# optuna/optuna

Measured on AMD Instinct MI355X. Metric: sampler suggest()/sec at 10k-trial history, 20-dim space, higher is better.
Workload: dtype fp64; 1 GPU; model=TPESampler multivariate Parzen-KDE + EI, history_trials=10000, dims=20, n_ei_candidates=24, parallelism=single, hip_kernels=True

## Files before the change

### optuna_amd/_hip/csrc/hipcore.hip

```cpp
#include "hip_common.h"

#include "gp_logei.h"
#include "mo_host.h"
#include "mo_rank.h"
#include "tpe_host.h"
#include "truncnorm_ops.h"

PYBIND11_MODULE(_hipcore, m) {
    m.doc() = "optuna_amd MI355X (gfx950) HIP kernels: TPE parzen fit + mixture "
              "log-pdf, truncnorm device library";
    m.def("available", &available);
    m.def("device_count", &device_count);
    m.def("log_gauss_mass", &log_gauss_mass);
    m.def("truncnorm_ppf", &truncnorm_ppf);
    m.def("truncnorm_logpdf", &truncnorm_logpdf);
    m.def("nondomination_rank", &nondomination_rank, py::arg("vals"),
          py::arg("n_below"));
    m.def("hv3d", &hv3d, py::arg("pts"), py::arg("ref_x"), py::arg("ref_y"),
          py::arg("ref_z"));
    py::class_<GpLogEiSession>(m, "GpLogEiSession")
        .def(py::init<int64_t, int64_t, int64_t, int64_t, int64_t, int64_t,
                      double, double, double>(),
             py::arg("X_ptr"), py::arg("alpha_ptr"), py::arg("cinv_ptr"),
             py::arg("eta_ptr"), py::arg("N"), py::arg("D"), py::arg("scale"),
             py::arg("stab_noise"), py::arg("threshold"))
        .def("eval", &GpLogEiSession::eval, py::arg("x"), py::arg("with_grad"));
    py::class_<Hssp3dSession>(m, "Hssp3dSession")
        .def(py::init<const arr_f64&, double, double, double>(), py::arg("cand"),
             py::arg("ref_x"), py::arg("ref_y"), py::arg("ref_z"))
        .def("round", &Hssp3dSession::round, py::arg("sx"), py::arg("sxz"),
             py::arg("sy"), py::arg("syz"), py::arg("syr"))
        .def("run", &Hssp3dSession::run, py::arg("subset_size"));
    m.def("hssp3d_contrib", &hssp3d_contrib, py::arg("cand"), py::arg("sx"),
          py::arg("sxz"), py::arg("sy"), py::arg("syz"), py::arg("syr"),
          py::arg("ref_x"), py::arg("ref_y"), py::arg("ref_z"));
    m.def("hv4d", &hv4d, py::arg("pts"), py::arg("ref_w"), py::arg("ref_x"),
          py::arg("ref_y"), py::arg("ref_z"));
    m.def("hssp4d_contrib", &hssp4d_contrib, py::arg("cand"), py::arg("sw"),
          py::arg("sx"), py::arg("sy"), py::arg("syz"), py::arg("syrw"),
          py::arg("syrx"), py::arg("ref_w"), py::arg("ref_x"), py::arg("ref_y"),
          py::arg("ref_z"));
    py::class_<Hssp4dSession>(m, "Hssp4dSession")
        .def(py::init<const arr_f64&, double, double, double, double>(),
             py::arg("cand"), py::arg("ref_w"), py::arg("ref_x"),
             py::arg("ref_y"), py::arg("ref_z"))
        .def("run", &Hssp4dSession::run, py::arg("subset_size"));
    m.attr("HSSP4D_MAX_SUBSET") = py::int_(HSSP4_MAX_K);
    m.def("kde_logpdf", &kde_logpdf, py::arg("obs"), py::arg("sorted_pos"),
          py::arg("logw"), py::arg("alow"), py::arg("ahigh"), py::arg("steps"),
          py::arg("n_choices"), py::arg("prior_weight"),
          py::arg("x"), py::arg("xedges"),
          py::arg("consider_endpoints") = false, py::arg("magic_clip") = true);
    m.def("tpe_below_kernels", &tpe_below_kernels, py::arg("obs"),
          py::arg("alow"), py::arg("ahigh"), py::arg("consider_endpoints"),
          py::arg("consider_magic_clip"), py::arg("active"));
    py::class_<TpeDeviceHistory>(m, "TpeDeviceHistory")
        .def(py::init<int64_t>(), py::arg("dims"))
        .def_property_readonly("n_rows", &TpeDeviceHistory::n_rows)
        .def("append", &TpeDeviceHistory::append, py::arg("block"))
        .def("upload_sorted", &TpeDeviceHistory::upload_sorted, py::arg("cols"))
        .def("insert_sorted", &TpeDeviceHistory::insert_sorted, py::arg("pos"),
             py::arg("rows"))
        .def_property_readonly("n_sorted", &TpeDeviceHistory::n_sorted)
        .def("insert_sorted_by_value", &TpeDeviceHistory::insert_sorted_by_value,
             py::arg("first_row"), py::arg("n_new"))
        .def("sorted_index", &TpeDeviceHistory::sorted_index)
        .def("set_domain", &TpeDeviceHistory::set_domain, py::arg("alow"),
             py::arg("ahigh"), py::arg("steps"), py::arg("n_choices"))
        .def("fused_prepare", &TpeDeviceHistory::fused_prepare, py::arg("excl"),
             py::arg("n_above"), py::arg("logw") = arr_f64(),
             py::arg("w_num") = 0, py::arg("w_start") = 1.0,
             py::arg("w_step") = 0.0, py::arg("log_total") = 0.0,
             py::arg("prior_weight") = 1.0,
             py::arg("consider_endpoints") = false,
             py::arg("magic_clip") = true)
        .def("fused_score", &TpeDeviceHistory::fused_score, py::arg("excl"),
             py::arg("n_above"), py::arg("x"), py::arg("xedges"),
             py::arg("bmu"), py::arg("bsig"), py::arg("bw"),
             py::arg("logw") = arr_f64(), py::arg("w_num") = 0,
             py::arg("w_start") = 1.0, py::arg("w_step") = 0.0,
             py::arg("log_total") = 0.0, py::arg("prior_weight") = 1.0,
             py::arg("consider_endpoints") = false,
             py::arg("magic_clip") = true, py::arg("return_parts") = false)
        .def("score", &TpeDeviceHistory::score, py::arg("sorted_rows"),
             py::arg("pos"), py::arg("n_above"), py::arg("logw"), py::arg("alow"),
             py::arg("ahigh"), py::arg("steps"), py::arg("n_choices"),
             py::arg("prior_weight"), py::arg("x"), py::arg("xedges"),
             py::arg("consider_endpoints") = false,
             py::arg("magic_clip") = true,
             py::arg("extras_raw") = arr_f64(),
             py::arg("extras_sorted") = arr_f64(),
             py::arg("extras_sorted_idx") = arr_i32(),
             py::arg("per_dim") = false);
}
```

### optuna_amd/_hip/csrc/tpe_host.h

```cpp
#pragma once

#include "hip_common.h"
#include "tpe_below_host.h"
#include "tpe_fused_kernels.h"
#include "tpe_kernels.h"

static void launch_mix_logpdf(hipStream_t st, const double* d_x,
                              const double* d_xedges, const double* d_c1,
                              const double* d_c2, const double* d_c3,
                              const double* d_logw, const double* d_steps,
                              const double* d_nchoices, double cat_base,
                              int64_t K, int64_t D, int64_t S, double* d_out,
                              double* d_scratch) {
    const int block = 256;
    const size_t shmem = (4 * (size_t)D + 2 * block) * sizeof(double);
    const int64_t n_chunks = mix_n_chunks(K);
    if (n_chunks <= 1) {
        hipLaunchKernelGGL(k_mix_logpdf, dim3((unsigned)S), dim3(block), shmem, st,
                           d_x, d_xedges, d_c1, d_c2, d_c3, d_logw, d_steps,
                           d_nchoices, cat_base, K, D, d_out);
        return;
    }
    double* d_part_m = d_scratch;
    double* d_part_s = d_scratch + (size_t)n_chunks * S;
    hipLaunchKernelGGL(k_mix_logpdf_partial, dim3((unsigned)S, (unsigned)n_chunks),
                       dim3(block), shmem, st, d_x, d_xedges, d_c1, d_c2, d_c3,
                       d_logw, d_steps, d_nchoices, cat_base, K, D, MIX_CHUNK,
                       d_part_m, d_part_s);
    hipLaunchKernelGGL(k_mix_logpdf_merge, dim3((unsigned)S), dim3(64), 0, st,
                       d_part_m, d_part_s, n_chunks, S, d_out);
}

py::array_t<double> kde_logpdf(const arr_f64& obs, const arr_i64& sorted_pos,
                               const arr_f64& logw, const arr_f64& alow,
                               const arr_f64& ahigh, const arr_f64& steps,
                               const arr_f64& n_choices, double prior_weight,
// ... 387 lines not shown

    void fused_prepare(const arr_i32& excl, int64_t n_above, const arr_f64& logw,
                       int64_t w_num, double w_start, double w_step,
                       double log_total, double prior_weight,
                       bool consider_endpoints, bool magic_clip) {
        check_fit_args("fused_prepare", excl, n_above, logw);
        g_ws.begin_uploads();
        launch_fit(excl, n_above, logw, w_num, w_start, w_step, log_total,
                   prior_weight, consider_endpoints, magic_clip,
                   true);
    }

    py::object fused_score(const arr_i32& excl, int64_t n_above,
                                    const arr_f64& x, const arr_f64& xedges,
                                    const arr_f64& bmu, const arr_f64& bsig,
                                    const arr_f64& bw, const arr_f64& logw,
                                    int64_t w_num, double w_start,
                                    double w_step, double log_total,
                                    double prior_weight,
                                    bool consider_endpoints, bool magic_clip,
                                    bool return_parts) {
        check_fit_args("fused_score", excl, n_above, logw);
        if (x.ndim() != 2 || x.shape(1) != D_ || bmu.ndim() != 2 ||
            bmu.shape(1) != D_ || bsig.ndim() != 2 || bsig.shape(1) != D_)
            throw std::runtime_error("fused_score: shape mismatch");
        const int64_t S = x.shape(0);
        const int64_t Kb = bmu.shape(0);
        const int64_t K = n_above + 1;
        if (S < 1 || Kb < 1 || Kb > FUSED_MAX_BELOW || bsig.shape(0) != Kb ||
            (int64_t)bw.size() != Kb ||
            (has_steps_ && (int64_t)xedges.size() != 2 * S * D_))
            throw std::runtime_error("fused_score: shape mismatch");

        hipStream_t st = g_ws.get_stream();
        g_ws.begin_uploads();
        if (!prepared_matches(excl, n_above, logw, w_num, w_start, w_step,
                              log_total, prior_weight, consider_endpoints,
                              magic_clip))
            launch_fit(excl, n_above, logw, w_num, w_start, w_step, log_total,
                       prior_weight, consider_endpoints, magic_clip,
                       false);

        const size_t n_x = (size_t)S * D_;
        const size_t n_b = (size_t)Kb * D_;
        const int64_t n_as = (K + SCORE_SLICE - 1) / SCORE_SLICE;
        const int64_t pass_dims = std::min<int64_t>(D_, SCORE_DC);
        const int below_slice = (int)std::max<int64_t>(
            1, std::min<int64_t>(SCORE_SLICE, SCORE_SLICE * SCORE_WAVES / pass_dims));
        const int64_t n_bs = (Kb + below_slice - 1) / below_slice;
        const size_t n_part = (size_t)(n_as + n_bs) * S;
        WsLayout L;
        const auto s_x = L.add<double>(n_x);
        const auto s_bmu = L.add<double>(n_b), s_bsig = L.add<double>(n_b);
        const auto s_bw = L.add<double>(Kb);
        const auto s_xedges = L.add<double>(has_steps_ ? 2 * n_x : 0);
        const size_t up_bytes = L.bytes();
        const auto s_part_m = L.add<double>(n_part), s_part_s = L.add<double>(n_part);
        char* base = g_ws.ensure_bytes(L.bytes());
        double *d_x = s_x.in(base), *d_bmu = s_bmu.in(base),
               *d_bsig = s_bsig.in(base), *d_bw = s_bw.in(base),
               *d_xedges = s_xedges.in(base), *d_part_m = s_part_m.in(base),
               *d_part_s = s_part_s.in(base);
        {
            char* h = g_ws.stage(up_bytes, st);
            memcpy(s_x.in(h), x.data(), n_x * 8);
            memcpy(s_bmu.in(h), bmu.data(), n_b * 8);
            memcpy(s_bsig.in(h), bsig.data(), n_b * 8);
            memcpy(s_bw.in(h), bw.data(), (size_t)Kb * 8);
            if (has_steps_) memcpy(s_xedges.in(h), xedges.data(), 2 * n_x * 8);
            HIP_CHECK(hipMemcpyAsync(base, h, up_bytes, hipMemcpyHostToDevice, st));
        }

        const CoefLayout C(K, D_, excl.size());
        const double* d_logw = C.logw.in(coef_.ptr);
        const int64_t n_groups = (S + SCORE_CAND - 1) / SCORE_CAND;
        hipLaunchKernelGGL(k_fused_score,
                           dim3((unsigned)(n_as + n_bs), (unsigned)n_groups),
                           dim3(SCORE_SLICE * SCORE_WAVES), 0, st, d_x, d_xedges,
                           C.c1.in(coef_.ptr), C.c2.in(coef_.ptr),
                           C.c3.in(coef_.ptr), d_logw, K, n_as,
                           d_bmu, d_bsig, d_bw, Kb, below_slice, domain_.ptr,
                           has_steps_ ? 1 : 0,
                           D_, S, d_part_m, d_part_s);
        const double* h_out =
            reinterpret_cast<const double*>(g_ws.stage(3 * (size_t)S * 8, st));
        hipLaunchKernelGGL(k_fused_merge, dim3((unsigned)S), dim3(64), 0, st,
                           d_part_m, d_part_s, n_as, n_bs, S,
                           const_cast<double*>(h_out));
        if (return_parts) {
            py::array_t<double> parts({(int64_t)3, S});
            py::array_t<double> lw(K);
            HIP_CHECK(hipMemcpyAsync(lw.mutable_data(), d_logw, (size_t)K * 8,
                                     hipMemcpyDeviceToHost, st));
            HIP_CHECK(hipStreamSynchronize(st));
            HIP_CHECK(hipGetLastError());
            memcpy(parts.mutable_data(), h_out, 3 * (size_t)S * 8);
            return py::make_tuple(parts, lw);
        }
        py::array_t<double> out(S);
        HIP_CHECK(hipStreamSynchronize(st));
        HIP_CHECK(hipGetLastError());
        memcpy(out.mutable_data(), h_out, (size_t)S * 8);
        return out;
    }

  private:
    struct PreparedFit {
        bool valid = false;
        int64_t n = 0, n_sorted = 0, Na = 0, w_num = 0;
        double w_start = 0.0, w_step = 0.0, log_total = 0.0, prior_weight = 0.0;
        bool consider_endpoints = false, magic_clip = false;
        std::vector<int32_t> excl;
        std::vector<double> logw;
    };

    void check_fit_args(const char* who, const arr_i32& excl, int64_t Na,
                        const arr_f64& logw) const {
        const std::string w(who);
        if (!sorted_valid_) throw std::runtime_error(w + " before upload_sorted");
        if (!domain_.ptr) throw std::runtime_error(w + " before set_domain");
        if (has_categorical_)
            throw std::runtime_error(w + ": categorical dims unsupported");
        const int64_t E = excl.size();
        const int64_t Nv = n_sorted_;
        if (E > FUSED_MAX_EXCL || Na < 0 || Na > Nv || Na + E < Nv ||
            (logw.size() > 0 && (int64_t)logw.size() != Na + 1))
            throw std::runtime_error(w + ": shape mismatch");
        const int32_t* ex = excl.data();
        for (int64_t e = 0; e < E; ++e)
            if (ex[e] < 0 || ex[e] >= n_ || (e > 0 && ex[e] <= ex[e - 1]))
                throw std::runtime_error(w + ": excl must be sorted table rows");
    }

    bool prepared_matches(const arr_i32& excl, int64_t Na, const arr_f64& logw,
                          int64_t w_num, double w_start, double w_step,
                          double log_total, double prior_weight,
                          bool consider_endpoints, bool magic_clip) const {
        const PreparedFit& p = prep_;
        const double a[4] = {w_start, w_step, log_total, prior_weight};
        const double b[4] = {p.w_start, p.w_step, p.log_total, p.prior_weight};
        return p.valid && p.n == n_ && p.n_sorted == n_sorted_ && p.Na == Na &&
               p.w_num == w_num && memcmp(a, b, sizeof(a)) == 0 &&
               p.consider_endpoints == consider_endpoints &&
               p.magic_clip == magic_clip &&
               p.excl.size() == (size_t)excl.size() &&
               (p.excl.empty() ||
                memcmp(p.excl.data(), excl.data(), p.excl.size() * 4) == 0) &&
               p.logw.size() == (size_t)logw.size() &&
               (p.logw.empty() ||
                memcmp(p.logw.data(), logw.data(), p.logw.size() * 8) == 0);
    }

    struct CoefLayout {
        WsLayout L;
        WsSlot<double> c1, c2, c3, logw;
        WsSlot<int32_t> excl;
        CoefLayout(int64_t K, int64_t D, int64_t E)
            : c1(L.add<double>((size_t)K * D)), c2(L.add<double>((size_t)K * D)),
              c3(L.add<double>((size_t)K * D)), logw(L.add<double>(K)),
              excl(L.add<int32_t>(E)) {}
    };

    void launch_fit(const arr_i32& excl, int64_t Na, const arr_f64& logw,
                    int64_t w_num, double w_start, double w_step,
// ... 37 lines not shown
        prep_.Na = Na;
        prep_.w_num = w_num;
        prep_.w_start = w_start;
        prep_.w_step = w_step;
        prep_.log_total = log_total;
        prep_.prior_weight = prior_weight;
        prep_.consider_endpoints = consider_endpoints;
        prep_.magic_clip = magic_clip;
        prep_.excl.assign(excl.data(), excl.data() + E);
        prep_.logw.assign(logw.data(), logw.data() + logw.size());
        prep_.valid = true;
    }

    void ensure_sorted_capacity(int64_t need, hipStream_t st) {
        if (need <= sorted_cap_) return;
        const int64_t new_cap = std::max<int64_t>(1024, need * 2);
        sorted_.grow_preserving((size_t)new_cap * D_, D_, n_sorted_, st);
        sorted_cap_ = new_cap;
    }

    int64_t D_;
    int64_t n_ = 0;
    int64_t capacity_ = 0;
    DeviceBuffer<double> params_;
    DeviceBuffer<int32_t> sorted_;
    int64_t n_sorted_ = 0;
    int64_t sorted_cap_ = 0;
    bool sorted_valid_ = false;
    DeviceBuffer<double> domain_;
    bool has_steps_ = false;
    bool has_categorical_ = false;
    DeviceBuffer<char> coef_;
    PreparedFit prep_;
};
```

### optuna_amd/samplers/_tpe/_device.py

```python
from __future__ import annotations

import math
import os
from typing import TYPE_CHECKING, NamedTuple

import numpy as np

from optuna_amd import _hip
from optuna_amd.distributions import (
    BaseDistribution,
    CategoricalDistribution,
    FloatDistribution,
    IntDistribution,
)
from optuna_amd.samplers._tpe import _truncnorm_np as _tn
from optuna_amd.samplers._tpe.parzen import _NumericalSpace, _to_param_domain


if TYPE_CHECKING:
    from optuna_amd.samplers._tpe._history import _SpaceCache

DEVICE_MIN_KERNELS = 512


# ... 42 lines not shown
    if n < 25:
        return 0, 1.0, 0.0, math.log(n + prior_weight) if n else 0.0
    num = n - 25
    start = 1.0 / n
    step = (1.0 - start) / (num - 1) if num > 1 else 0.0
    if num > 1:
        ramp_sum = num * (start + 1.0) / 2.0
    else:
        ramp_sum = start * num
    return num, start, step, math.log(ramp_sum + 25.0 + prior_weight)


def expand_weight_ramp(n: int, prior_weight: float) -> np.ndarray:
    num, start, step, _ = default_weight_ramp(n, prior_weight)
    w = np.ones(n + 1, dtype=np.float64)
    k = np.arange(num, dtype=np.float64)
    w[:num] = k * step + start
    if num > 1:
        w[num - 1] = 1.0
    w[n] = prior_weight if n else 1.0
    return w


def native_below_enabled() -> bool:
    return os.environ.get("OPTUNA_AMD_TPE_NATIVE_BELOW", "1") != "0"


_UNRESOLVED = object()


def native_below(cache: "_SpaceCache"):
    if not native_below_enabled():
        return None
    fn = getattr(cache, "_native_below", _UNRESOLVED)
    if fn is _UNRESOLVED:
        fn = getattr(_hip.get(), "tpe_below_kernels", None)
        cache._native_below = fn
    return fn


def draw_below_native(
    fn,
    cache: "_SpaceCache",
    below_rows: np.ndarray,
    weights: np.ndarray,
    rng: np.random.RandomState,
    size: int,
    consider_endpoints: bool,
    consider_magic_clip: bool,
) -> tuple[np.ndarray, np.ndarray, np.ndarray]:
    ns = getattr(cache, "_numerical_space", None)
    if ns is None:
        ns = cache._numerical_space = _NumericalSpace.of(cache.dists)
    obs = cache.params[below_rows[cache.valid[below_rows]]]
    if ns.is_log.any():
        obs[:, ns.is_log] = np.log(obs[:, ns.is_log])
    active = rng.choice(len(weights), p=weights, size=size)
    mus, sigmas, a, b, loc, scale = fn(
        obs, ns.adapted_lows, ns.adapted_highs, consider_endpoints, consider_magic_clip, active
    )
    q = rng.uniform(low=0, high=1, size=a.shape)
    x = _tn.ppf(q, a, b) * scale + loc
    _to_param_domain(x, ns.kinds, ns.lows, ns.highs, ns.steps)
    return x, mus, sigmas


class FusedRequest(NamedTuple):

    below_rows: np.ndarray
    n_above: int
    x_raw: np.ndarray
    below_mus: np.ndarray
    below_sigmas: np.ndarray
    below_weights: np.ndarray


def _space_domains(
    space: dict[str, BaseDistribution],
) -> tuple[np.ndarray, np.ndarray, np.ndarray, np.ndarray]:
    dists = list(space.values())
    is_cat = np.array([isinstance(d, CategoricalDistribution) for d in dists])
    is_log = np.array(
        [False if c else bool(d.log) for c, d in zip(is_cat, dists)]
    )
    steps = np.array(
        [
            0.0 if c else (float(d.step) if d.step is not None else 0.0)
            for c, d in zip(is_cat, dists)
        ],
        dtype=np.float64,
    )
    n_choices = np.array(
        [float(len(d.choices)) if c else 0.0 for c, d in zip(is_cat, dists)],
        dtype=np.float64,
    )
    alow = np.zeros(len(dists))
    ahigh = np.ones(len(dists))
# ... 199 lines not shown
            cache, req.below_rows, req.n_above, weights, consider_endpoints,
            consider_magic_clip, prior_weight,
        )
        if self._prepared is None or self._prepared[0] != self._suggest_key(*args):
            self.prepare_fused(*args)
        assert self._prepared is not None
        fit_args, self._prepared = self._prepared[1], None
        excl, n_above, logw, w_num, w_start, w_step, log_total = fit_args[:7]
        x = req.x_raw
        xedges = _cell_edges(x, self._is_log, self._steps) if self._has_steps else _EMPTY_F64
        if self._is_log.any():
            x = x.copy()
            x[:, self._is_log] = np.log(x[:, self._is_log])
        return self._hist.fused_score(
            excl,
            n_above,
            x,
            xedges,
            req.below_mus,
            req.below_sigmas,
            req.below_weights,
            logw,
            w_num,
            w_start,
            w_step,
            log_total,
            float(prior_weight),
            consider_endpoints,
            consider_magic_clip,
            return_parts,
        )


def _mirror_of(cache: "_SpaceCache") -> _SpaceDeviceMirror:
    mirror = getattr(cache, "_device_mirror", None)
    if mirror is None:
        mirror = _SpaceDeviceMirror(cache.space)
        cache._device_mirror = mirror
    return mirror


def prepare_fused_resident(
    cache: "_SpaceCache",
    below_rows: np.ndarray,
    n_above: int,
    weights: np.ndarray | None,
    consider_endpoints: bool,
    consider_magic_clip: bool,
    prior_weight: float = 1.0,
) -> None:
    if not _hip.is_available():
        return
    _mirror_of(cache).prepare_fused(
        cache, below_rows, n_above, weights, consider_endpoints, consider_magic_clip,
        prior_weight,
    )


def score_above_resident(
    cache: "_SpaceCache",
    sel: np.ndarray | None,
    weights: np.ndarray | None,
    samples: dict[str, np.ndarray] | None,
    consider_endpoints: bool,
    consider_magic_clip: bool,
    prior_weight: float = 1.0,
    extras: np.ndarray | None = None,
    per_dim: bool = False,
    fused: FusedRequest | None = None,
) -> np.ndarray:
    mirror = _mirror_of(cache)
    if fused is not None:
        return mirror.score_fused(
            cache, fused, weights, consider_endpoints, consider_magic_clip, prior_weight
        )
    return mirror.score(
        cache, sel, weights, samples, consider_endpoints, consider_magic_clip,
        prior_weight=prior_weight, extras=extras, per_dim=per_dim,
    )


def kde_logpdf(
    space: dict[str, BaseDistribution],
    observations: dict[str, np.ndarray],
    orders: dict[str, np.ndarray] | None,
    weights: np.ndarray,
    samples: dict[str, np.ndarray],
    consider_endpoints: bool,
    consider_magic_clip: bool,
    prior_weight: float = 1.0,
) -> np.ndarray:
    core = _hip.get()
    assert core is not None
    names = list(space.keys())
    D = len(names)
    N = len(observations[names[0]])

    is_log, alow, ahigh, steps, n_choices = _space_domains(space)
    obs = np.empty((N, D), dtype=np.float64)
    x_raw = np.column_stack(
        [np.asarray(samples[n], dtype=np.float64) for n in names]
    )
    sorted_pos = np.empty((N, D), dtype=np.int64)
    for c, name in enumerate(names):
# ... 29 lines not shown
```

### optuna_amd/samplers/_tpe/sampler.py

```python
from __future__ import annotations

import json
import math
from typing import TYPE_CHECKING, Any, Callable, Sequence

import numpy as np

from optuna_amd import logging as _logging
from optuna_amd.distributions import BaseDistribution
from optuna_amd.samplers._base import (
    _INDEPENDENT_SAMPLING_WARNING_TEMPLATE,
    BaseSampler,
    _process_constraints_after_trial,
)
from optuna_amd.samplers._lazy_random_state import LazyRandomState
from optuna_amd.samplers._random import RandomSampler
from optuna_amd.samplers._tpe.parzen import (
    _mixture_weights,
    _ParzenEstimator,
    _ParzenEstimatorParameters,
)
from optuna_amd.search_space import IntersectionSearchSpace
from optuna_amd.search_space.group_decomposed import (
    _GroupDecomposedSearchSpace,
# ... 388 lines not shown
                                for name, dist in search_space.items()
                            ]
                        )
                if rows_list:
                    liar_extras = np.asarray(rows_list, dtype=np.float64)
        n_liar = 0 if liar_extras is None else len(liar_extras)

        n_below_valid = int(np.count_nonzero(cache.valid[below_rows]))
        fused = _device.fused_eligible(
            search_space,
            per_dim=per_dim,
            n_liar=n_liar,
            default_estimator=self._parzen_estimator_cls is _ParzenEstimator,
            rows_ascending=history._rows_number_ascending,
            n_excl=len(below_rows) + cache.n_invalid,
            n_below_kernels=n_below_valid + 1,
        )
        if fused:
            n_above = cache.n_valid - n_below_valid
        else:
            if above_sel is None:
                above_sel = history.valid_rows(search_space, above_rows, cache)
            n_above = len(above_sel)

        use_device = (
            self._parzen_estimator_cls is _ParzenEstimator
            and _device.space_is_device_eligible(search_space)
            and _device.device_ready(n_above + n_liar + 1)
        )
        fused = fused and use_device
        fused_weights: np.ndarray | None = None
        below_native = None
        p = self._parzen_estimator_parameters
        if fused and p.weights is default_weights and p.prior_weight >= 0:
            below_native = _device.native_below(cache)
        if fused:
            if p.weights is not default_weights:
                fused_weights = self._above_weights(n_above)
            _device.prepare_fused_resident(
                cache,
                below_rows,
                n_above,
                fused_weights,
                p.consider_endpoints,
                p.consider_magic_clip,
                prior_weight=p.prior_weight,
            )

        obs_above: dict[str, np.ndarray] = {}
        orders_above: dict[str, np.ndarray] | None = None
        if not use_device:
            obs_above, orders_above = history.observations(search_space, above_rows, cache)
            if n_liar:
                assert liar_extras is not None
                obs_above = {
                    name: np.concatenate([obs_above[name], liar_extras[:, c]])
                    for c, name in enumerate(search_space)
                }
                orders_above = None

        if below_native is not None:
            below_weights = self._below_weights(n_below_valid, study._is_multi_objective())
            x_below, below_mus, below_sigmas = _device.draw_below_native(
                below_native,
                cache,
                below_rows,
                below_weights,
                self._rng.rng,
                self._n_ei_candidates,
                p.consider_endpoints,
                p.consider_magic_clip,
            )
            samples_below = {name: x_below[:, i] for i, name in enumerate(cache.names)}
        else:
            obs_below, orders_below = history.observations(search_space, below_rows, cache)
            mpe_below = self._build_mpe(
                study, search_space, obs_below, handle_below=True, orders=orders_below
            )
            if per_dim:
                samples_below = mpe_below.sample_per_dim(self._rng.rng, self._n_ei_candidates)
            elif fused:
                x_below = mpe_below._sample_array(self._rng.rng, self._n_ei_candidates)
                samples_below = {
                    name: x_below[:, i] for i, name in enumerate(mpe_below._param_names)
                }
                below_mus = mpe_below._numerical.mus
                below_sigmas = mpe_below._numerical.sigmas
                below_weights = mpe_below.weights
            else:
                samples_below = mpe_below.sample(self._rng.rng, self._n_ei_candidates)

        if fused:
            acq_func_vals = _device.score_above_resident(
                cache,
                None,
# ... 340 lines not shown
```

Measured before the change: 2306 suggest/s.

## Fuse below-KDE candidate drawing, truncnorm ppf and scoring into one native call

```diff
diff --git a/optuna_amd/_hip/csrc/hipcore.hip b/optuna_amd/_hip/csrc/hipcore.hip
--- a/optuna_amd/_hip/csrc/hipcore.hip
+++ b/optuna_amd/_hip/csrc/hipcore.hip
@@ -54,6 +54,7 @@
     m.def("tpe_below_kernels", &tpe_below_kernels, py::arg("obs"),
           py::arg("alow"), py::arg("ahigh"), py::arg("consider_endpoints"),
           py::arg("consider_magic_clip"), py::arg("active"));
+    tpe_draw_py::register_functions(m, (size_t)FUSED_MAX_BELOW);
     py::class_<TpeDeviceHistory>(m, "TpeDeviceHistory")
         .def(py::init<int64_t>(), py::arg("dims"))
         .def_property_readonly("n_rows", &TpeDeviceHistory::n_rows)
@@ -82,6 +83,17 @@
              py::arg("log_total") = 0.0, py::arg("prior_weight") = 1.0,
              py::arg("consider_endpoints") = false,
              py::arg("magic_clip") = true, py::arg("return_parts") = false)
+        .def("fused_draw_score", &TpeDeviceHistory::fused_draw_score,
+             py::arg("excl"), py::arg("n_above"), py::arg("table"),
+             py::arg("valid"), py::arg("below_rows"), py::arg("bw"),
+             py::arg("u"), py::arg("q"), py::arg("alow"), py::arg("ahigh"),
+             py::arg("kinds"), py::arg("lows"), py::arg("highs"),
+             py::arg("steps"), py::arg("logw") = arr_f64(),
+             py::arg("w_num") = 0, py::arg("w_start") = 1.0,
+             py::arg("w_step") = 0.0, py::arg("log_total") = 0.0,
+             py::arg("prior_weight") = 1.0,
+             py::arg("consider_endpoints") = false,
+             py::arg("magic_clip") = true)
         .def("score", &TpeDeviceHistory::score, py::arg("sorted_rows"),
              py::arg("pos"), py::arg("n_above"), py::arg("logw"), py::arg("alow"),
              py::arg("ahigh"), py::arg("steps"), py::arg("n_choices"),
diff --git a/optuna_amd/_hip/csrc/tpe_draw_bind.h b/optuna_amd/_hip/csrc/tpe_draw_bind.h
--- /dev/null
+++ b/optuna_amd/_hip/csrc/tpe_draw_bind.h
@@ -0,0 +1,251 @@
+#pragma once
+
+#include <pybind11/numpy.h>
+#include <pybind11/pybind11.h>
+
+#include <cstring>
+#include <stdexcept>
+#include <string>
+#include <vector>
+
+#include "tpe_below_host.h"
+#include "tpe_draw_host.h"
+
+namespace tpe_draw_py {
+
+namespace py = pybind11;
+
+constexpr const char* SCALAR_SIG = "double (double, int __pyx_skip_dispatch)";
+
+struct Binding {
+    tpe_draw::Ops ops;
+    py::object log, log1p, exp, logaddexp;
+    py::object owner;
+    bool bound = false;
+};
+
+inline Binding& binding() {
+    static Binding* b = new Binding();
+    return *b;
+}
+
+inline py::array view(const double* p, size_t n) {
+    return py::array(py::dtype::of<double>(), {(py::ssize_t)n},
+                     {(py::ssize_t)sizeof(double)}, p, binding().owner);
+}
+
+inline void call_unary(const py::object& uf, const double* in, double* out,
+                       size_t n) {
+    uf(view(in, n), view(out, n));
+}
+
+inline bool bind(const py::object& ndtr, const py::object& log_ndtr,
+                 const py::object& ndtri_exp) {
+    Binding& B = binding();
+    using scalar_fn = double (*)(double, int);
+    scalar_fn fns[3] = {nullptr, nullptr, nullptr};
+    const py::object* caps[3] = {&ndtr, &log_ndtr, &ndtri_exp};
+    for (int i = 0; i < 3; ++i) {
+        PyObject* c = caps[i]->ptr();
+        const char* name = PyCapsule_CheckExact(c) ? PyCapsule_GetName(c) : nullptr;
+        void* p = nullptr;
+        if (name != nullptr && std::strcmp(name, SCALAR_SIG) == 0)
+            p = PyCapsule_GetPointer(c, name);
+        if (p == nullptr) {
+            PyErr_Clear();
+            B.bound = false;
+            return false;
+        }
+        fns[i] = reinterpret_cast<scalar_fn>(p);
+    }
+    if (B.bound && B.ops.ndtr == fns[0] && B.ops.log_ndtr == fns[1] &&
+        B.ops.ndtri_exp == fns[2])
+        return true;
+    B.bound = false;
+    py::module_ np = py::module_::import("numpy");
+    B.log = np.attr("log");
+    B.log1p = np.attr("log1p");
+    B.exp = np.attr("exp");
+    B.logaddexp = np.attr("logaddexp");
+    B.owner = py::none();
+    B.ops.ndtr = fns[0];
+    B.ops.log_ndtr = fns[1];
+    B.ops.ndtri_exp = fns[2];
+    B.ops.ctx = &B;
+    B.ops.log = [](void* c, const double* in, double* out, size_t n) {
+        call_unary(static_cast<Binding*>(c)->log, in, out, n);
+    };
+    B.ops.log1p = [](void* c, const double* in, double* out, size_t n) {
+        call_unary(static_cast<Binding*>(c)->log1p, in, out, n);
+    };
+    B.ops.exp = [](void* c, const double* in, double* out, size_t n) {
+        call_unary(static_cast<Binding*>(c)->exp, in, out, n);
+    };
+    B.ops.logaddexp = [](void* c, const double* x, const double* y, double* out,
+                         size_t n) {
+        static_cast<Binding*>(c)->logaddexp(view(x, n), view(y, n), view(out, n));
+    };
+    B.bound = true;
+    return true;
+}
+
+inline bool bound() { return binding().bound; }
+
+inline const tpe_draw::Ops& ops() {
+    if (!binding().bound) throw std::runtime_error("tpe_draw: not bound");
+    return binding().ops;
+}
+
+template <typename T>
+const T* typed(const py::array& arr, const char* name, py::ssize_t ndim) {
+    if (!py::isinstance<py::array_t<T>>(arr) || !(arr.flags() & py::array::c_style) ||
+        arr.ndim() != ndim)
+        throw std::runtime_error(std::string("tpe_draw: ") + name +
+                                 " has the wrong dtype, rank or layout");
+    return static_cast<const T*>(arr.data());
+}
+
+struct HostDraw {
+    size_t n = 0, D = 0, S = 0;
+    std::vector<double> obs, mus, sigmas, a, b, loc, scale, p, x_raw, x_kde,
+        xedges;
+    std::vector<int64_t> active;
+    tpe_draw::Workspace ws;
+    size_t Kb() const { return n + 1; }
+};
+
+inline void draw(HostDraw& H, const py::array& table, const py::array& valid,
+                 const py::array& below_rows, const py::array& bw,
+                 const py::array& u, const py::array& q, const py::array& alow,
+                 const py::array& ahigh, const py::array& kinds,
+                 const py::array& lows, const py::array& highs,
+                 const py::array& steps, bool consider_endpoints,
+                 bool consider_magic_clip, bool with_edges, size_t max_kernels) {
+    const tpe_draw::Ops& op = ops();
+    const double* p_table = typed<double>(table, "table", 2);
+    const bool* p_valid = typed<bool>(valid, "valid", 1);
+    const int64_t* p_rows = typed<int64_t>(below_rows, "below_rows", 1);
+    const double* p_bw = typed<double>(bw, "bw", 1);
+    const double* p_u = typed<double>(u, "u", 1);
+    const double* p_q = typed<double>(q, "q", 2);
+    const double* p_alow = typed<double>(alow, "alow", 1);
+    const double* p_ahigh = typed<double>(ahigh, "ahigh", 1);
+    const int8_t* p_kinds = typed<int8_t>(kinds, "kinds", 1);
+    const double* p_lows = typed<double>(lows, "lows", 1);
+    const double* p_highs = typed<double>(highs, "highs", 1);
+    const double* p_steps = typed<double>(steps, "steps", 1);
+    const py::ssize_t N = table.shape(0), D = table.shape(1), S = u.shape(0);
+    if (D < 1 || S < 1 || valid.shape(0) != N || q.shape(0) != S ||
+        q.shape(1) != D || alow.shape(0) != D || ahigh.shape(0) != D ||
+        kinds.shape(0) != D || lows.shape(0) != D || highs.shape(0) != D ||
+        steps.shape(0) != D)
+        throw std::runtime_error("tpe_draw: shape mismatch");
+    for (py::ssize_t c = 0; c < D; ++c)
+        if (p_kinds[c] < tpe_draw::KIND_CONT || p_kinds[c] > tpe_draw::KIND_LOG_DISC)
+            throw std::runtime_error("tpe_draw: numerical dims only");
+
+    const py::ssize_t m = below_rows.shape(0);
+    H.D = (size_t)D;
+    H.S = (size_t)S;
+    H.obs.resize((size_t)m * D);
+    size_t n = 0;
+    for (py::ssize_t i = 0; i < m; ++i) {
+        const int64_t r = p_rows[i];
+        if (r < 0 || r >= N) throw std::runtime_error("tpe_draw: below row out of range");
+        if (!p_valid[r]) continue;
+        std::memcpy(&H.obs[n * D], p_table + (size_t)r * D, (size_t)D * 8);
+        ++n;
+    }
+    H.n = n;
+    if (n + 1 > max_kernels) throw std::runtime_error("tpe_draw: too many below kernels");
+    if ((size_t)bw.shape(0) != n + 1)
+        throw std::runtime_error("tpe_draw: one weight per below kernel expected");
+    tpe_draw::log_observations(op, H.obs.data(), n, (size_t)D, p_kinds, H.ws);
+
+    H.active.resize((size_t)S);
+    tpe_draw::choose(p_bw, n + 1, p_u, (size_t)S, H.active.data(), H.ws);
+    for (py::ssize_t s = 0; s < S; ++s)
+        if (H.active[s] < 0 || (size_t)H.active[s] > n)
+            throw std::runtime_error("tpe_draw: weights do not form a distribution");
+
+    const size_t n_k = (n + 1) * (size_t)D, n_x = (size_t)S * D;
+    H.mus.resize(n_k);
+    H.sigmas.resize(n_k);
+    for (auto* v : {&H.a, &H.b, &H.loc, &H.scale, &H.p, &H.x_raw, &H.x_kde})
+        v->resize(n_x);
+    H.xedges.resize(with_edges ? 2 * n_x : 0);
+    tpe_below::fit_and_gather(H.obs.data(), n, (size_t)D, p_alow, p_ahigh,
+                              consider_endpoints, consider_magic_clip,
+                              H.active.data(), (size_t)S, H.mus.data(),
+                              H.sigmas.data(), H.a.data(), H.b.data(),
+                              H.loc.data(), H.scale.data());
+    tpe_draw::ppf(op, p_q, H.a.data(), H.b.data(), n_x, H.p.data(), H.ws);
+    tpe_draw::to_candidates(op, H.p.data(), H.loc.data(), H.scale.data(),
+                            (size_t)S, (size_t)D, p_kinds, p_lows, p_highs,
+                            p_steps, H.x_raw.data(), H.x_kde.data(),
+                            with_edges ? H.xedges.data() : nullptr, H.ws);
+}
+
+inline py::array_t<double> copy_out(const std::vector<double>& v, size_t rows,
+                                    size_t cols) {
+    py::array_t<double> out({(py::ssize_t)rows, (py::ssize_t)cols});
+    if (rows * cols != 0) std::memcpy(out.mutable_data(), v.data(), rows * cols * 8);
+    return out;
+}
+
+inline void register_functions(py::module_& m, size_t max_kernels) {
+    m.def("tpe_draw_bind", &bind, py::arg("ndtr"), py::arg("log_ndtr"),
+          py::arg("ndtri_exp"));
+    m.def("tpe_draw_bound", &bound);
+    m.def("tpe_draw_ppf", [](const py::array& q, const py::array& a,
+                             const py::array& b) {
+        const double* pq = typed<double>(q, "q", q.ndim());
+        const double* pa = typed<double>(a, "a", q.ndim());
+        const double* pb = typed<double>(b, "b", q.ndim());
+        if (a.size() != q.size() || b.size() != q.size())
+            throw std::runtime_error("tpe_draw_ppf: shape mismatch");
+        py::array_t<double> out(std::vector<py::ssize_t>(q.shape(), q.shape() + q.ndim()));
+        tpe_draw::Workspace ws;
+        tpe_draw::ppf(ops(), pq, pa, pb, (size_t)q.size(), out.mutable_data(), ws);
+        return out;
+    });
+    m.def("tpe_draw_choice", [](const py::array& w, const py::array& u) {
+        const double* pw = typed<double>(w, "w", 1);
+        const double* pu = typed<double>(u, "u", 1);
+        py::array_t<int64_t> out(u.shape(0));
+        tpe_draw::Workspace ws;
+        tpe_draw::choose(pw, (size_t)w.shape(0), pu, (size_t)u.shape(0),
+                         out.mutable_data(), ws);
+        return out;
+    });
+    m.def("tpe_draw_argmax", [](const py::array& v) {
+        const double* pv = typed<double>(v, "v", 1);
+        if (v.shape(0) < 1) throw std::runtime_error("tpe_draw_argmax: empty");
+        return tpe_draw::argmax(pv, (size_t)v.shape(0));
+    });
+    m.def(
+        "tpe_draw_candidates",
+        [max_kernels](const py::array& table, const py::array& valid,
+                      const py::array& below_rows, const py::array& bw,
+                      const py::array& u, const py::array& q,
+                      const py::array& alow, const py::array& ahigh,
+                      const py::array& kinds, const py::array& lows,
+                      const py::array& highs, const py::array& steps,
+                      bool consider_endpoints, bool consider_magic_clip) {
+            HostDraw H;
+            draw(H, table, valid, below_rows, bw, u, q, alow, ahigh, kinds, lows,
+                 highs, steps, consider_endpoints, consider_magic_clip, true,
+                 max_kernels);
+            return py::make_tuple(copy_out(H.x_raw, H.S, H.D),
+                                  copy_out(H.mus, H.Kb(), H.D),
+                                  copy_out(H.sigmas, H.Kb(), H.D),
+                                  copy_out(H.x_kde, H.S, H.D),
+                                  copy_out(H.xedges, H.S, 2 * H.D));
+        },
+        py::arg("table"), py::arg("valid"), py::arg("below_rows"), py::arg("bw"),
+        py::arg("u"), py::arg("q"), py::arg("alow"), py::arg("ahigh"),
+        py::arg("kinds"), py::arg("lows"), py::arg("highs"), py::arg("steps"),
+        py::arg("consider_endpoints"), py::arg("consider_magic_clip"));
+}
+
+}
diff --git a/optuna_amd/_hip/csrc/tpe_draw_host.h b/optuna_amd/_hip/csrc/tpe_draw_host.h
--- /dev/null
+++ b/optuna_amd/_hip/csrc/tpe_draw_host.h
@@ -0,0 +1,261 @@
+#pragma once
+
+#include <algorithm>
+#include <cmath>
+#include <cstddef>
+#include <cstdint>
+#include <limits>
+#include <vector>
+
+#if defined(__clang__)
+#define TPE_DRAW_FP_CONTRACT_OFF _Pragma("clang fp contract(off)")
+#elif defined(__GNUC__)
+#define TPE_DRAW_FP_CONTRACT_OFF
+#pragma GCC push_options
+#pragma GCC optimize("fp-contract=off")
+#else
+#define TPE_DRAW_FP_CONTRACT_OFF _Pragma("STDC FP_CONTRACT OFF")
+#endif
+
+namespace tpe_draw {
+
+constexpr int8_t KIND_CONT = 0, KIND_LOG = 1, KIND_DISC = 2, KIND_LOG_DISC = 3;
+
+struct Ops {
+    double (*ndtr)(double, int) = nullptr;
+    double (*log_ndtr)(double, int) = nullptr;
+    double (*ndtri_exp)(double, int) = nullptr;
+    void (*log)(void* ctx, const double* in, double* out, size_t n) = nullptr;
+    void (*log1p)(void* ctx, const double* in, double* out, size_t n) = nullptr;
+    void (*exp)(void* ctx, const double* in, double* out, size_t n) = nullptr;
+    void (*logaddexp)(void* ctx, const double* x, const double* y, double* out,
+                      size_t n) = nullptr;
+    void* ctx = nullptr;
+};
+
+struct Workspace {
+    std::vector<double> f[9];
+    std::vector<uint32_t> at[3];
+    double* get(int i, size_t n) {
+        if (f[i].size() < n) f[i].resize(n);
+        return f[i].data();
+    }
+    uint32_t* idx(int i, size_t n) {
+        if (at[i].size() < n) at[i].resize(n);
+        return at[i].data();
+    }
+};
+
+inline double np_clip(double x, double lo, double hi) {
+    if (x != x) return x;
+    const double t = x > lo ? x : lo;
+    if (t != t) return t;
+    return t < hi ? t : hi;
+}
+
+inline void choose(const double* w, size_t n, const double* u, size_t S,
+                   int64_t* active, Workspace& ws) {
+    TPE_DRAW_FP_CONTRACT_OFF
+    if (n == 0) return;
+    double* cdf = ws.get(0, n);
+    cdf[0] = w[0];
+    for (size_t i = 1; i < n; ++i) cdf[i] = cdf[i - 1] + w[i];
+    const double total = cdf[n - 1];
+    for (size_t i = 0; i < n; ++i) cdf[i] /= total;
+    for (size_t s = 0; s < S; ++s)
+        active[s] = (int64_t)(std::upper_bound(cdf, cdf + n, u[s]) - cdf);
+}
+
+inline void ppf(const Ops& op, const double* q, const double* a, const double* b,
+                size_t n, double* out, Workspace& ws) {
+    TPE_DRAW_FP_CONTRACT_OFF
+    if (n == 0) return;
+    const double ninf = -std::numeric_limits<double>::infinity();
+    double* lx = ws.get(0, n);
+    double* ly = ws.get(1, n);
+    double* mass = ws.get(2, n);
+    double* e_in = ws.get(3, n);
+    double* e_out = ws.get(4, n);
+    double* p_in = ws.get(5, 2 * n);
+    double* p_out = ws.get(6, 2 * n);
+    double* g_in = ws.get(7, n);
+    double* g_out = ws.get(8, n);
+    uint32_t* e_at = ws.idx(0, n);
+    uint32_t* p_at = ws.idx(1, 2 * n);
+    uint32_t* g_at = ws.idx(2, n);
+    size_t ne = 0, np = 0, ng = 0;
+
+    for (size_t i = 0; i < n; ++i) {
+        const double ai = a[i], bi = b[i];
+        const bool left = ai < 0;
+        if (left) {
+            g_in[ng] = q[i];
+            g_at[ng++] = (uint32_t)i;
+        }
+        if (!(ai < bi)) {
+            mass[i] = ninf;
+            lx[i] = left ? op.log_ndtr(ai, 0) : op.log_ndtr(-bi, 0);
+        } else if (ai > 0) {
+            const double lb = op.log_ndtr(-ai, 0);
+            const double t = op.log_ndtr(-bi, 0);
+            e_in[ne] = t - lb;
+            e_at[ne++] = (uint32_t)i;
+            mass[i] = lb;
+            lx[i] = t;
+        } else if (bi <= 0) {
+            const double lb = op.log_ndtr(bi, 0);
+            const double t = op.log_ndtr(ai, 0);
+            e_in[ne] = t - lb;
+            e_at[ne++] = (uint32_t)i;
+            mass[i] = lb;
+            lx[i] = t;
+        } else {
+            p_in[np] = -op.ndtr(ai, 0) - op.ndtr(-bi, 0);
+            p_at[np++] = (uint32_t)i;
+            lx[i] = left ? op.log_ndtr(ai, 0) : op.log_ndtr(-bi, 0);
+        }
+    }
+    const size_t n_central = np;
+    if (ne) op.exp(op.ctx, e_in, e_out, ne);
+    for (size_t k = 0; k < ne; ++k) {
+        p_in[np] = -e_out[k];
+        p_at[np++] = e_at[k];
+    }
+    const size_t n_mass = np;
+    for (size_t i = 0; i < n; ++i)
+        if (!(a[i] < 0)) {
+            p_in[np] = -q[i];
+            p_at[np++] = (uint32_t)i;
+        }
+    if (np) op.log1p(op.ctx, p_in, p_out, np);
+    if (ng) op.log(op.ctx, g_in, g_out, ng);
+    for (size_t k = 0; k < n_central; ++k) mass[p_at[k]] = p_out[k];
+    for (size_t k = n_central; k < n_mass; ++k)
+        mass[p_at[k]] = mass[p_at[k]] + p_out[k];
+    for (size_t k = n_mass; k < np; ++k) ly[p_at[k]] = p_out[k] + mass[p_at[k]];
+    for (size_t k = 0; k < ng; ++k) ly[g_at[k]] = g_out[k] + mass[g_at[k]];
+    double* r = e_in;
+    op.logaddexp(op.ctx, lx, ly, r, n);
+    for (size_t i = 0; i < n; ++i) {
+        const double ai = a[i], bi = b[i];
+        const double v = ai < 0 ? op.ndtri_exp(r[i], 0) : -op.ndtri_exp(r[i], 0);
+        out[i] = ai >= bi ? std::numeric_limits<double>::quiet_NaN()
+                          : np_clip(v, ai, bi);
+    }
+}
+
+inline void log_observations(const Ops& op, double* obs, size_t n, size_t D,
+                             const int8_t* kinds, Workspace& ws) {
+    size_t n_log = 0;
+    for (size_t c = 0; c < D; ++c)
+        n_log += kinds[c] == KIND_LOG || kinds[c] == KIND_LOG_DISC;
+    if (n_log == 0 || n == 0) return;
+    double* in = ws.get(0, n * n_log);
+    double* out = ws.get(1, n * n_log);
+    size_t k = 0;
+    for (size_t r = 0; r < n; ++r)
+        for (size_t c = 0; c < D; ++c)
+            if (kinds[c] == KIND_LOG || kinds[c] == KIND_LOG_DISC)
+                in[k++] = obs[r * D + c];
+    op.log(op.ctx, in, out, k);
+    k = 0;
+    for (size_t r = 0; r < n; ++r)
+        for (size_t c = 0; c < D; ++c)
+            if (kinds[c] == KIND_LOG || kinds[c] == KIND_LOG_DISC)
+                obs[r * D + c] = out[k++];
+}
+
+inline void to_candidates(const Ops& op, const double* p, const double* loc,
+                          const double* scale, size_t S, size_t D,
+                          const int8_t* kinds, const double* lows,
+                          const double* highs, const double* steps,
+                          double* x_raw, double* x_kde, double* xedges,
+                          Workspace& ws) {
+    TPE_DRAW_FP_CONTRACT_OFF
+    const size_t n = S * D;
+    size_t n_log = 0, n_log_step = 0;
+    for (size_t c = 0; c < D; ++c) {
+        const bool is_log = kinds[c] == KIND_LOG || kinds[c] == KIND_LOG_DISC;
+        n_log += is_log;
+        n_log_step += is_log && steps[c] > 0 && xedges != nullptr;
+    }
+    for (size_t i = 0; i < n; ++i) x_raw[i] = p[i] * scale[i] + loc[i];
+    const auto is_log = [&](size_t c) {
+        return kinds[c] == KIND_LOG || kinds[c] == KIND_LOG_DISC;
+    };
+    double* in = ws.get(0, S * (n_log + 2 * n_log_step));
+    double* out = ws.get(1, S * (n_log + 2 * n_log_step));
+    if (n_log) {
+        size_t k = 0;
+        for (size_t s = 0; s < S; ++s)
+            for (size_t c = 0; c < D; ++c)
+                if (is_log(c)) in[k++] = x_raw[s * D + c];
+        op.exp(op.ctx, in, out, k);
+        k = 0;
+        for (size_t s = 0; s < S; ++s)
+            for (size_t c = 0; c < D; ++c)
+                if (is_log(c)) x_raw[s * D + c] = out[k++];
+    }
+    for (size_t c = 0; c < D; ++c) {
+        if (!(steps[c] > 0)) continue;
+        const double lo = lows[c], hi = highs[c], st = steps[c];
+        for (size_t s = 0; s < S; ++s) {
+            const double v = x_raw[s * D + c];
+            x_raw[s * D + c] =
+                np_clip(lo + std::nearbyint((v - lo) / st) * st, lo, hi);
+        }
+    }
+    for (size_t i = 0; i < n; ++i) x_kde[i] = x_raw[i];
+    if (xedges != nullptr) {
+        for (size_t i = 0; i < 2 * n; ++i) xedges[i] = 0.0;
+        for (size_t c = 0; c < D; ++c) {
+            if (!(steps[c] > 0)) continue;
+            const double half = steps[c] / 2;
+            for (size_t s = 0; s < S; ++s) {
+                xedges[s * 2 * D + c] = x_raw[s * D + c] - half;
+                xedges[s * 2 * D + D + c] = x_raw[s * D + c] + half;
+            }
+        }
+    }
+    if (n_log) {
+        size_t k = 0;
+        for (size_t s = 0; s < S; ++s)
+            for (size_t c = 0; c < D; ++c)
+                if (is_log(c)) in[k++] = x_raw[s * D + c];
+        if (n_log_step)
+            for (size_t s = 0; s < S; ++s)
+                for (size_t c = 0; c < D; ++c)
+                    if (is_log(c) && steps[c] > 0) {
+                        in[k++] = xedges[s * 2 * D + c];
+                        in[k++] = xedges[s * 2 * D + D + c];
+                    }
+        op.log(op.ctx, in, out, k);
+        k = 0;
+        for (size_t s = 0; s < S; ++s)
+            for (size_t c = 0; c < D; ++c)
+                if (is_log(c)) x_kde[s * D + c] = out[k++];
+        if (n_log_step)
+            for (size_t s = 0; s < S; ++s)
+                for (size_t c = 0; c < D; ++c)
+                    if (is_log(c) && steps[c] > 0) {
+                        xedges[s * 2 * D + c] = out[k++];
+                        xedges[s * 2 * D + D + c] = out[k++];
+                    }
+    }
+}
+
+inline size_t argmax(const double* v, size_t n) {
+    size_t best = 0;
+    for (size_t i = 0; i < n; ++i) {
+        if (v[i] != v[i]) return i;
+        if (v[i] > v[best]) best = i;
+    }
+    return best;
+}
+
+}
+
+#if !defined(__clang__) && defined(__GNUC__)
+#pragma GCC pop_options
+#endif
+#undef TPE_DRAW_FP_CONTRACT_OFF
diff --git a/optuna_amd/_hip/csrc/tpe_host.h b/optuna_amd/_hip/csrc/tpe_host.h
--- a/optuna_amd/_hip/csrc/tpe_host.h
+++ b/optuna_amd/_hip/csrc/tpe_host.h
@@ -2,6 +2,7 @@
 
 #include "hip_common.h"
 #include "tpe_below_host.h"
+#include "tpe_draw_bind.h"
 #include "tpe_fused_kernels.h"
 #include "tpe_kernels.h"
 
@@ -455,6 +456,91 @@
             (has_steps_ && (int64_t)xedges.size() != 2 * S * D_))
             throw std::runtime_error("fused_score: shape mismatch");
 
+        py::array_t<double> lw(return_parts ? K : 0);
+        py::array_t<double> out(return_parts ? 0 : S);
+        const double* h_out = score_candidates(
+            excl, n_above, x.data(), xedges.data(), bmu.data(), bsig.data(),
+            bw.data(), S, Kb, logw, w_num, w_start, w_step, log_total,
+            prior_weight, consider_endpoints, magic_clip,
+            return_parts ? lw.mutable_data() : nullptr);
+        if (return_parts) {
+            py::array_t<double> parts({(int64_t)3, S});
+            memcpy(parts.mutable_data(), h_out, 3 * (size_t)S * 8);
+            return py::make_tuple(parts, lw);
+        }
+        memcpy(out.mutable_data(), h_out, (size_t)S * 8);
+        return out;
+    }
+
+    py::tuple fused_draw_score(const arr_i32& excl, int64_t n_above,
+                               const py::array& table, const py::array& valid,
+                               const py::array& below_rows, const py::array& bw,
+                               const py::array& u, const py::array& q,
+                               const py::array& alow, const py::array& ahigh,
+                               const py::array& kinds, const py::array& lows,
+                               const py::array& highs, const py::array& steps,
+                               const arr_f64& logw, int64_t w_num,
+                               double w_start, double w_step, double log_total,
+                               double prior_weight, bool consider_endpoints,
+                               bool magic_clip) {
+        check_fit_args("fused_draw_score", excl, n_above, logw);
+        if (table.ndim() != 2 || table.shape(1) != D_)
+            throw std::runtime_error("fused_draw_score: shape mismatch");
+        tpe_draw_py::HostDraw& H = draw_;
+        tpe_draw_py::draw(H, table, valid, below_rows, bw, u, q, alow, ahigh,
+                          kinds, lows, highs, steps, consider_endpoints,
+                          magic_clip, has_steps_, (size_t)FUSED_MAX_BELOW);
+        const int64_t S = (int64_t)H.S;
+        py::array_t<double> out(S);
+        py::array_t<double> x_raw = tpe_draw_py::copy_out(H.x_raw, H.S, H.D);
+        const double* h_out = score_candidates(
+            excl, n_above, H.x_kde.data(), H.xedges.data(), H.mus.data(),
+            H.sigmas.data(), static_cast<const double*>(bw.data()), S,
+            (int64_t)H.Kb(), logw, w_num, w_start, w_step, log_total,
+            prior_weight, consider_endpoints, magic_clip, nullptr);
+        memcpy(out.mutable_data(), h_out, (size_t)S * 8);
+        const size_t best = tpe_draw::argmax(h_out, (size_t)S);
+        return py::make_tuple(best, x_raw, out);
+    }
+
+  private:
+    struct PreparedFit {
+        bool valid = false;
+        int64_t n = 0, n_sorted = 0, Na = 0, w_num = 0;
+        double w_start = 0.0, w_step = 0.0, log_total = 0.0, prior_weight = 0.0;
+        bool consider_endpoints = false, magic_clip = false;
+        std::vector<int32_t> excl;
+        std::vector<double> logw;
+    };
+
+    void check_fit_args(const char* who, const arr_i32& excl, int64_t Na,
+                        const arr_f64& logw) const {
+        const std::string w(who);
+        if (!sorted_valid_) throw std::runtime_error(w + " before upload_sorted");
+        if (!domain_.ptr) throw std::runtime_error(w + " before set_domain");
+        if (has_categorical_)
+            throw std::runtime_error(w + ": categorical dims unsupported");
+        const int64_t E = excl.size();
+        const int64_t Nv = n_sorted_;
+        if (E > FUSED_MAX_EXCL || Na < 0 || Na > Nv || Na + E < Nv ||
+            (logw.size() > 0 && (int64_t)logw.size() != Na + 1))
+            throw std::runtime_error(w + ": shape mismatch");
+        const int32_t* ex = excl.data();
+        for (int64_t e = 0; e < E; ++e)
+            if (ex[e] < 0 || ex[e] >= n_ || (e > 0 && ex[e] <= ex[e - 1]))
+                throw std::runtime_error(w + ": excl must be sorted table rows");
+    }
+
+    const double* score_candidates(const arr_i32& excl, int64_t n_above,
+                                   const double* x, const double* xedges,
+                                   const double* bmu, const double* bsig,
+                                   const double* bw, int64_t S, int64_t Kb,
+                                   const arr_f64& logw, int64_t w_num,
+                                   double w_start, double w_step,
+                                   double log_total, double prior_weight,
+                                   bool consider_endpoints, bool magic_clip,
+                                   double* lw_out) {
+        const int64_t K = n_above + 1;
         hipStream_t st = g_ws.get_stream();
         g_ws.begin_uploads();
         if (!prepared_matches(excl, n_above, logw, w_num, w_start, w_step,
@@ -486,11 +572,11 @@
                *d_part_s = s_part_s.in(base);
         {
             char* h = g_ws.stage(up_bytes, st);
-            memcpy(s_x.in(h), x.data(), n_x * 8);
-            memcpy(s_bmu.in(h), bmu.data(), n_b * 8);
-            memcpy(s_bsig.in(h), bsig.data(), n_b * 8);
-            memcpy(s_bw.in(h), bw.data(), (size_t)Kb * 8);
-            if (has_steps_) memcpy(s_xedges.in(h), xedges.data(), 2 * n_x * 8);
+            memcpy(s_x.in(h), x, n_x * 8);
+            memcpy(s_bmu.in(h), bmu, n_b * 8);
+            memcpy(s_bsig.in(h), bsig, n_b * 8);
+            memcpy(s_bw.in(h), bw, (size_t)Kb * 8);
+            if (has_steps_) memcpy(s_xedges.in(h), xedges, 2 * n_x * 8);
             HIP_CHECK(hipMemcpyAsync(base, h, up_bytes, hipMemcpyHostToDevice, st));
         }
 
@@ -510,49 +596,12 @@
         hipLaunchKernelGGL(k_fused_merge, dim3((unsigned)S), dim3(64), 0, st,
                            d_part_m, d_part_s, n_as, n_bs, S,
                            const_cast<double*>(h_out));
-        if (return_parts) {
-            py::array_t<double> parts({(int64_t)3, S});
-            py::array_t<double> lw(K);
-            HIP_CHECK(hipMemcpyAsync(lw.mutable_data(), d_logw, (size_t)K * 8,
+        if (lw_out != nullptr)
+            HIP_CHECK(hipMemcpyAsync(lw_out, d_logw, (size_t)K * 8,
                                      hipMemcpyDeviceToHost, st));
-            HIP_CHECK(hipStreamSynchronize(st));
-            HIP_CHECK(hipGetLastError());
-            memcpy(parts.mutable_data(), h_out, 3 * (size_t)S * 8);
-            return py::make_tuple(parts, lw);
-        }
-        py::array_t<double> out(S);
         HIP_CHECK(hipStreamSynchronize(st));
         HIP_CHECK(hipGetLastError());
-        memcpy(out.mutable_data(), h_out, (size_t)S * 8);
-        return out;
-    }
-
-  private:
-    struct PreparedFit {
-        bool valid = false;
-        int64_t n = 0, n_sorted = 0, Na = 0, w_num = 0;
-        double w_start = 0.0, w_step = 0.0, log_total = 0.0, prior_weight = 0.0;
-        bool consider_endpoints = false, magic_clip = false;
-        std::vector<int32_t> excl;
-        std::vector<double> logw;
-    };
-
-    void check_fit_args(const char* who, const arr_i32& excl, int64_t Na,
-                        const arr_f64& logw) const {
-        const std::string w(who);
-        if (!sorted_valid_) throw std::runtime_error(w + " before upload_sorted");
-        if (!domain_.ptr) throw std::runtime_error(w + " before set_domain");
-        if (has_categorical_)
-            throw std::runtime_error(w + ": categorical dims unsupported");
-        const int64_t E = excl.size();
-        const int64_t Nv = n_sorted_;
-        if (E > FUSED_MAX_EXCL || Na < 0 || Na > Nv || Na + E < Nv ||
-            (logw.size() > 0 && (int64_t)logw.size() != Na + 1))
-            throw std::runtime_error(w + ": shape mismatch");
-        const int32_t* ex = excl.data();
-        for (int64_t e = 0; e < E; ++e)
-            if (ex[e] < 0 || ex[e] >= n_ || (e > 0 && ex[e] <= ex[e - 1]))
-                throw std::runtime_error(w + ": excl must be sorted table rows");
+        return h_out;
     }
 
     bool prepared_matches(const arr_i32& excl, int64_t Na, const arr_f64& logw,
@@ -656,4 +705,5 @@
     bool has_categorical_ = false;
     DeviceBuffer<char> coef_;
     PreparedFit prep_;
+    tpe_draw_py::HostDraw draw_;
 };
diff --git a/optuna_amd/samplers/_tpe/_device.py b/optuna_amd/samplers/_tpe/_device.py
--- a/optuna_amd/samplers/_tpe/_device.py
+++ b/optuna_amd/samplers/_tpe/_device.py
@@ -98,6 +98,8 @@
 def native_below(cache: "_SpaceCache"):
     if not native_below_enabled():
         return None
+    if native_draw(cache):
+        return cache._native_draw_entry
     fn = getattr(cache, "_native_below", _UNRESOLVED)
     if fn is _UNRESOLVED:
         fn = getattr(_hip.get(), "tpe_below_kernels", None)
@@ -115,9 +117,7 @@
     consider_endpoints: bool,
     consider_magic_clip: bool,
 ) -> tuple[np.ndarray, np.ndarray, np.ndarray]:
-    ns = getattr(cache, "_numerical_space", None)
-    if ns is None:
-        ns = cache._numerical_space = _NumericalSpace.of(cache.dists)
+    ns = _numerical_space_of(cache)
     obs = cache.params[below_rows[cache.valid[below_rows]]]
     if ns.is_log.any():
         obs[:, ns.is_log] = np.log(obs[:, ns.is_log])
@@ -129,6 +129,58 @@
     x = _tn.ppf(q, a, b) * scale + loc
     _to_param_domain(x, ns.kinds, ns.lows, ns.highs, ns.steps)
     return x, mus, sigmas
+
+
+def native_draw_enabled() -> bool:
+    return os.environ.get("OPTUNA_AMD_TPE_NATIVE_DRAW", "1") != "0"
+
+
+def _draw_capsules() -> tuple | None:
+    try:
+        from scipy.special import cython_special
+
+        capi = cython_special.__pyx_capi__
+        return capi["__pyx_fuse_1ndtr"], capi["__pyx_fuse_1log_ndtr"], capi["ndtri_exp"]
+    except (ImportError, AttributeError, KeyError):
+        return None
+
+
+def _bind_native_draw(core) -> bool:
+    bind = getattr(core, "tpe_draw_bind", None)
+    capsules = _draw_capsules() if bind is not None else None
+    return capsules is not None and bool(bind(*capsules))
+
+
+def native_draw(cache: "_SpaceCache") -> bool:
+    if not native_draw_enabled():
+        return False
+    entry = getattr(cache, "_native_draw_entry", _UNRESOLVED)
+    if entry is _UNRESOLVED:
+        mirror = getattr(cache, "_device_mirror", None)
+        if mirror is None:
+            return False
+        entry = getattr(mirror._hist, "fused_draw_score", None)
+        if entry is not None and not _bind_native_draw(_hip.get()):
+            entry = None
+        cache._native_draw_entry = entry
+    return entry is not None
+
+
+def _numerical_space_of(cache: "_SpaceCache") -> _NumericalSpace:
+    ns = getattr(cache, "_numerical_space", None)
+    if ns is None:
+        ns = cache._numerical_space = _NumericalSpace.of(cache.dists)
+    return ns
+
+
+class DrawRequest(NamedTuple):
+
+    below_rows: np.ndarray
+    n_above: int
+    below_weights: np.ndarray
+    u: np.ndarray
+    q: np.ndarray
+    entry: object
 
 
 class FusedRequest(NamedTuple):
@@ -394,6 +446,51 @@
         )
 
 
+    def draw_score_fused(
+        self,
+        cache: "_SpaceCache",
+        req: DrawRequest,
+        consider_endpoints: bool,
+        consider_magic_clip: bool,
+        prior_weight: float,
+    ) -> tuple[int, np.ndarray, np.ndarray]:
+        args = (
+            cache, req.below_rows, req.n_above, None, consider_endpoints,
+            consider_magic_clip, prior_weight,
+        )
+        if self._prepared is None or self._prepared[0] != self._suggest_key(*args):
+            self.prepare_fused(*args)
+        assert self._prepared is not None
+        fit_args, self._prepared = self._prepared[1], None
+        excl, n_above, logw, w_num, w_start, w_step, log_total = fit_args[:7]
+        ns = _numerical_space_of(cache)
+        with np.errstate(divide="ignore", invalid="ignore"):
+            return req.entry(
+                excl,
+                n_above,
+                cache.params,
+                cache.valid,
+                np.ascontiguousarray(req.below_rows, dtype=np.int64),
+                req.below_weights,
+                req.u,
+                req.q,
+                ns.adapted_lows,
+                ns.adapted_highs,
+                ns.kinds,
+                ns.lows,
+                ns.highs,
+                ns.steps,
+                logw,
+                w_num,
+                w_start,
+                w_step,
+                log_total,
+                float(prior_weight),
+                consider_endpoints,
+                consider_magic_clip,
+            )
+
+
 def _mirror_of(cache: "_SpaceCache") -> _SpaceDeviceMirror:
     mirror = getattr(cache, "_device_mirror", None)
     if mirror is None:
@@ -429,9 +526,13 @@
     prior_weight: float = 1.0,
     extras: np.ndarray | None = None,
     per_dim: bool = False,
-    fused: FusedRequest | None = None,
-) -> np.ndarray:
+    fused: FusedRequest | DrawRequest | None = None,
+) -> np.ndarray | tuple[int, np.ndarray, np.ndarray]:
     mirror = _mirror_of(cache)
+    if isinstance(fused, DrawRequest):
+        return mirror.draw_score_fused(
+            cache, fused, consider_endpoints, consider_magic_clip, prior_weight
+        )
     if fused is not None:
         return mirror.score_fused(
             cache, fused, weights, consider_endpoints, consider_magic_clip, prior_weight
diff --git a/optuna_amd/samplers/_tpe/sampler.py b/optuna_amd/samplers/_tpe/sampler.py
--- a/optuna_amd/samplers/_tpe/sampler.py
+++ b/optuna_amd/samplers/_tpe/sampler.py
@@ -444,8 +444,6 @@
         fused_weights: np.ndarray | None = None
         below_native = None
         p = self._parzen_estimator_parameters
-        if fused and p.weights is default_weights and p.prior_weight >= 0:
-            below_native = _device.native_below(cache)
         if fused:
             if p.weights is not default_weights:
                 fused_weights = self._above_weights(n_above)
@@ -458,6 +456,8 @@
                 p.consider_magic_clip,
                 prior_weight=p.prior_weight,
             )
+            if p.weights is default_weights and p.prior_weight >= 0:
+                below_native = _device.native_below(cache)
 
         obs_above: dict[str, np.ndarray] = {}
         orders_above: dict[str, np.ndarray] | None = None
@@ -473,6 +473,28 @@
 
         if below_native is not None:
             below_weights = self._below_weights(n_below_valid, study._is_multi_objective())
+            if self._n_ei_candidates > 0 and _device.native_draw(cache):
+                u = self._rng.rng.random_sample(self._n_ei_candidates)
+                q = self._rng.rng.uniform(
+                    low=0, high=1, size=(self._n_ei_candidates, len(cache.names))
+                )
+                best, x_below, _ = _device.score_above_resident(
+                    cache,
+                    None,
+                    None,
+                    None,
+                    p.consider_endpoints,
+                    p.consider_magic_clip,
+                    prior_weight=p.prior_weight,
+                    fused=_device.DrawRequest(
+                        below_rows, n_above, below_weights, u, q, below_native
+                    ),
+                )
+                chosen = dict(zip(cache.names, x_below[best].tolist()))
+                return {
+                    name: dist.to_external_repr(chosen[name])
+                    for name, dist in search_space.items()
+                }
             x_below, below_mus, below_sigmas = _device.draw_below_native(
                 below_native,
                 cache,
```

New measurement: 2778 suggest/s (median of 6 runs). 1.2x the previous value.
